# kobby-pentangeli/chaum-pedersen-zkp

Measured on AMD Instinct MI355X. Metric: verified proofs/sec (1/2/4/8 MI355X) + % int-VALU roofline vs host-CPU, higher is better.
Workload: dtype int32/int64 limbs (GF(2^255-19), radix 2^25.5)

## Files before the change

### chaum-pedersen-zkp_amd/build_native.py

```python
from __future__ import annotations

import os
import shutil
import subprocess
import sys
from concurrent.futures import ThreadPoolExecutor

PKG = os.path.dirname(os.path.abspath(__file__))
ROOT = os.path.dirname(PKG)
CSRC = os.path.join(PKG, "csrc")
LIBDIR = os.path.join(PKG, "lib")
LIBCPZ = os.path.join(LIBDIR, "libcpz.so")
HOSTTEST = os.path.join(ROOT, "tests", "native", "libcpz_hosttest.so")
DEVPROBE = os.path.join(ROOT, "tests", "native", "libcpz_devprobe.so")
ARCH = os.environ.get("CPZ_OFFLOAD_ARCH", "gfx950")


def _hipcc() -> str:
    for cand in (shutil.which("hipcc"), "/opt/rocm/bin/hipcc"):
        if cand and os.path.exists(cand):
            return cand
    raise RuntimeError("hipcc not found: the gfx950 build needs ROCm")


def _newer(out: str, srcs) -> bool:
    if not os.path.exists(out):
        return True
    t = os.path.getmtime(out)
    return any(os.path.getmtime(s) > t for s in srcs)


def _headers():
    hdr = [os.path.join(CSRC, f) for f in os.listdir(CSRC) if f.endswith(".h")]
    return hdr + [os.path.join(ROOT, "include", "cpz.h")]


def _run(cmd):
    r = subprocess.run(cmd, stdout=subprocess.PIPE, stderr=subprocess.STDOUT, text=True)
    if r.returncode != 0:
        raise RuntimeError("build step failed: %s\n%s" % (" ".join(cmd), r.stdout[-4000:]))
    return r.stdout


UNIT_FLAGS = {"wide.hip": ["-falign-loops=64"]}


def build_libcpz(force: bool = False, verbose: bool = False, out: str = LIBCPZ, defines=()) -> str:
    units = ["kernels.hip", "wide.hip", "rlc.hip", "part.hip", "runtime.hip"]
    srcs = [os.path.join(CSRC, u) for u in units] + _headers()
    if not force and not defines and not _newer(out, srcs):
        return out
    objdir = os.path.join(os.path.dirname(out), "obj" if not defines else "obj_" + "_".join(defines).replace("=", ""))
    os.makedirs(objdir, exist_ok=True)
    hipcc = _hipcc()
    common = [hipcc, "--offload-arch=" + ARCH, "-O3", "-std=c++17", "-fPIC", "-I", CSRC,
              "-I", os.path.join(ROOT, "include")] + ["-D" + d for d in defines]
    if defines and os.environ.get("CPZ_EXTRA_FLAGS"):
        common += os.environ["CPZ_EXTRA_FLAGS"].split()

    def compile_one(u):
        obj = os.path.join(objdir, u.replace(".hip", ".o"))
        if force or defines or _newer(obj, [os.path.join(CSRC, u)] + _headers()):
            uf = [] if defines and os.environ.get("CPZ_NO_UNIT_FLAGS") else UNIT_FLAGS.get(u, [])
            _run(common + uf + ["-c", os.path.join(CSRC, u), "-o", obj])
        return obj

    with ThreadPoolExecutor(max_workers=len(units)) as ex:
        objs = list(ex.map(compile_one, units))
    tmp = out + ".tmp"
    _run([hipcc, "--offload-arch=" + ARCH, "-shared", "-fPIC", "-o", tmp] + objs)
    os.replace(tmp, out)
    if verbose:
        print("built", out)
    return out


CLOCK_PROBE_LIB = os.path.join(LIBDIR, "timing", "clock_probe.so")


def build_clock_probe(force: bool = False) -> str:
    os.makedirs(os.path.dirname(CLOCK_PROBE_LIB), exist_ok=True)
    return build_libcpz(force, out=CLOCK_PROBE_LIB, defines=("CPZ_CLOCK_PROBE", "CPZ_TIMING_ONLY"))


def build_hosttest(force: bool = False) -> str:
    src = os.path.join(ROOT, "tests", "native", "hostlib.cpp")
    if not force and not _newer(HOSTTEST, [src] + _headers()):
        return HOSTTEST
    cxx = shutil.which("g++") or "g++"
    tmp = HOSTTEST + ".tmp"
    extra = ["-D" + d for d in os.environ.get("CPZ_HOST_DEFINES", "").split()]
    _run([cxx, "-O2", "-std=c++17", "-fPIC", "-shared", "-DCPZ_BOUNDS_CHECK", "-DCPZ_COUNT_OPS"] + extra +
         ["-I", CSRC, src, "-o", tmp])
    os.replace(tmp, HOSTTEST)
    return HOSTTEST


def build_devprobe(force: bool = False, out: str = DEVPROBE, include: str = CSRC) -> str:
    src = os.path.join(ROOT, "tests", "native", "devprobe.hip")
    hdrs = [os.path.join(include, f) for f in os.listdir(include) if f.endswith(".h")]
    if not force and not _newer(out, [src] + hdrs):
        return out
    tmp = out + ".tmp"
    _run([_hipcc(), "--offload-arch=" + ARCH, "-O3", "-std=c++17", "-fPIC", "-I", include,
          "-I", os.path.join(ROOT, "include"), "-shared", src, "-o", tmp])
    os.replace(tmp, out)
    return out


CPP_TEST = os.path.join(ROOT, "tests", "cpp", "batch_verifier_test")


def build_cpp_test(force: bool = False) -> str:
    src = os.path.join(ROOT, "tests", "cpp", "batch_verifier_test.cpp")
    hdrs = [os.path.join(ROOT, "include", "cpz.h"), os.path.join(ROOT, "include", "cpz_batch.hpp")]
    if not force and not _newer(CPP_TEST, [src] + hdrs):
        return CPP_TEST
    cxx = shutil.which("g++") or "g++"
    _run([cxx, "-O2", "-std=c++17", "-I", os.path.join(ROOT, "include"), src, "-o", CPP_TEST + ".tmp",
          "-L", LIBDIR, "-lcpz", "-Wl,-rpath,$ORIGIN/../../chaum-pedersen-zkp_amd/lib"])
    os.replace(CPP_TEST + ".tmp", CPP_TEST)
    return CPP_TEST


DROPIN_TEST = os.path.join(ROOT, "tests", "cpp", "dropin_test")


def build_dropin_test(force: bool = False) -> str:
    src = os.path.join(ROOT, "tests", "cpp", "dropin_test.cpp")
    hdrs = [os.path.join(ROOT, "include", "cpz.h"), os.path.join(ROOT, "include", "cpz_batch.hpp")]
    if not force and not _newer(DROPIN_TEST, [src] + hdrs):
        return DROPIN_TEST
    cxx = shutil.which("g++") or "g++"
    _run([cxx, "-O2", "-std=c++17", "-I", os.path.join(ROOT, "include"), src, "-o", DROPIN_TEST + ".tmp",
          "-L", LIBDIR, "-lcpz", "-Wl,-rpath,$ORIGIN/../../chaum-pedersen-zkp_amd/lib"])
    os.replace(DROPIN_TEST + ".tmp", DROPIN_TEST)
    return DROPIN_TEST


MERGE_TEST = os.path.join(ROOT, "tests", "cpp", "merge_groups_test")


def build_merge_groups_test(force: bool = False) -> str:
    src = os.path.join(ROOT, "tests", "cpp", "merge_groups_test.cpp")
    hdrs = [os.path.join(ROOT, "include", "cpz.h"), os.path.join(ROOT, "include", "cpz_batch.hpp")]
    if not force and not _newer(MERGE_TEST, [src] + hdrs):
        return MERGE_TEST
    cxx = shutil.which("g++") or "g++"
    _run([cxx, "-O2", "-std=c++17", "-I", os.path.join(ROOT, "include"), src, "-o", MERGE_TEST + ".tmp",
          "-L", LIBDIR, "-lcpz", "-Wl,-rpath,$ORIGIN/../../chaum-pedersen-zkp_amd/lib"])
    os.replace(MERGE_TEST + ".tmp", MERGE_TEST)
    return MERGE_TEST


def build_oracle(force: bool = False) -> None:
    mk = os.path.join(ROOT, "oracle", "Makefile")
    if os.path.exists(mk):
        _run(["make", "-s", "-C", os.path.join(ROOT, "oracle")] + (["-B"] if force else []))


def build_all(force: bool = False, verbose: bool = False) -> None:
    build_hosttest(force)
    build_oracle(force)
    build_libcpz(force, verbose)
    build_devprobe(force)
    build_cpp_test(force)
    build_dropin_test(force)
    build_merge_groups_test(force)


if __name__ == "__main__":
    build_all(force="--force" in sys.argv, verbose=True)
```

### chaum-pedersen-zkp_amd/csrc/cpz_kernels.h

```cpp
#pragma once
#include <hip/hip_runtime.h>
#include <stdint.h>

#include "scalarmul.h"

namespace cpz {

constexpr uint8_t kStatusOk = 0;
constexpr uint8_t kStatusEqFail = 1;
constexpr uint8_t kStatusBadPoint = 2;
constexpr uint8_t kStatusBadScalar = 3;
constexpr uint8_t kStatusIdentity = 4;
constexpr uint8_t kStatusZeroS = 5;

constexpr int kNielsEntries = kTableB;
constexpr int kNielsLevels = 8;
__host__ __device__ constexpr int niels_level_doublings(int level) {
  return level == 0 ? 0 : (level == 1 ? 128 : (level == 2 ? 64 : (level == 3 ? 192 : 32 * (2 * (level - 4) + 1))));
}
constexpr int kNielsLevelOfPart[8] = {0, 4, 2, 5, 1, 6, 3, 7};
constexpr bool niels_parts_consistent() {
  for (int q = 0; q < 8; q++)
    if (niels_level_doublings(kNielsLevelOfPart[q]) != 32 * q) return false;
  return true;
}
static_assert(niels_parts_consistent(), "kNielsLevelOfPart must invert niels_level_doublings");
constexpr int kCachedEntries = 2 * kTableSlots;
#ifndef CPZ_VERIFY_BLOCK
#define CPZ_VERIFY_BLOCK 256
#endif
constexpr int kVerifyBlock = CPZ_VERIFY_BLOCK;

struct StrobeSnap {
  uint8_t state[200];
  int32_t pos;
  int32_t pos_begin;
  int32_t flags;
  int32_t pad;
};

struct ChallengeArgs {
  int64_t n;
  uint32_t gh_words[16];
  const uint32_t* y1;
  const uint32_t* y2;
  const uint32_t* r1;
  const uint32_t* r2;
  const uint32_t* s;
  const uint8_t* ctx_bytes;
  const uint64_t* ctx_off;
  const uint8_t* ctx_present;
  const uint64_t* ctx_end = nullptr;
  const StrobeSnap* prefix;
  uint32_t* c_out;
  uint8_t* status_out;
  int fast_noctx = 0;
  uint32_t k1[50];
  uint32_t k2[50];
  int fast_ctx32 = 0;
  uint32_t c32[3][50];
  int eq_only = 0;
};

enum ParseCode : uint8_t {
  kParseOk = 0, kParseTooSmall, kParseBadVersion,
  kParseR1LenMissing, kParseR1LenInvalid, kParseR1Truncated, kParseR1Size, kParseR1Point,
  kParseR2LenMissing, kParseR2LenInvalid, kParseR2Truncated, kParseR2Size, kParseR2Point,
  kParseSLenMissing, kParseSLenInvalid, kParseSTruncated, kParseSSize, kParseSScalar,
  kParseTrailing, kParseIdentity, kParseZeroS
};

struct ParseArgs {
  int64_t n;
  const uint8_t* blob;
  const uint64_t* off;
  uint32_t* r1;
  uint32_t* r2;
  uint32_t* s;
  uint8_t* code;
  uint32_t* aux;
};

constexpr int kProbeChunks = 16;
struct ProbeGatherArgs {
  int64_t starts[kProbeChunks];
  int blk;
  const uint32_t* rows[5];
  uint32_t* out_rows[5];
  const uint64_t* ctx_off;
  const uint8_t* ctx_present;
  uint64_t* out_begin;
  uint64_t* out_end;
  uint8_t* out_present;
};

#ifndef CPZ_VERIFY_QUAD
#define CPZ_VERIFY_QUAD 1
#endif
#ifndef CPZ_QUAD_MAX
#define CPZ_QUAD_MAX 16384
#endif
constexpr int64_t kQuadVerifyMax = CPZ_QUAD_MAX;
constexpr int kQuadTableInts = 2 * 9 * 40;
constexpr int64_t kVarBaseMax = kQuadVerifyMax;
constexpr int kQuadPhases = 9;
constexpr int kSmallStamps = 16;
constexpr int64_t kQuadProofScratch = 2 * kQuadTableInts * 4;

struct VerifyArgs {
  int64_t n;
  const uint32_t* y1;
  const uint32_t* y2;
  const uint32_t* r1;
  const uint32_t* r2;
  const uint32_t* s;
  const uint32_t* c;
  uint8_t* status;
  const ge_niels* comb;
  char* scratch;
  const ge_niels* pre = nullptr;
  int eq_only = 0;
  const uint32_t* blocks = nullptr;
  int block_proofs = 0;
  int64_t nblocks = 0;
  int64_t quad_max = 0;
  uint64_t* clock_probe = nullptr;
  const int32_t* vtab16 = nullptr;
  const ge_niels* vtab = nullptr;
};

struct PairDesc {
  const ge_niels* tab;
  const int32_t* tab16;
  StrobeSnap prefix[2];
  uint32_t gh_words[16];
  int32_t fast_noctx;
  int32_t fast_ctx32;
  uint32_t k1[50];
  uint32_t k2[50];
  uint32_t c32[3][50];
};
static_assert(sizeof(PairDesc) % 16 == 0, "descriptor rows stay 16-byte aligned");
struct PairArgs {
  const PairDesc* desc = nullptr;
  const uint32_t* pair_idx = nullptr;
};

struct ProveArgs {
  int64_t n;
  uint64_t first_index;
  uint32_t seed_x[8];
  uint32_t seed_k[8];
  const uint32_t* x_in;
  const uint32_t* k_in;
  const ge_niels* comb;
  uint32_t* y1;
  uint32_t* y2;
  uint32_t* r1;
  uint32_t* r2;
  const uint32_t* c;
  uint32_t* s_out;
};

hipError_t launch_transcript_prefix(const uint32_t* gh_words, StrobeSnap* out, hipStream_t st);
hipError_t launch_challenge(const ChallengeArgs& a, hipStream_t st);
hipError_t launch_probe_gather(const ProbeGatherArgs& a, hipStream_t st);
bool challenge_prefix_is_fixed(const StrobeSnap& snap);
bool challenge_prefix_is_ctx32(const StrobeSnap& snap);
hipError_t launch_build_niels(const uint32_t* base_words, int nbases, ge_niels* tab, int* ok, ge_p3* bases,
                              hipStream_t st);
hipError_t launch_niels_r16(const ge_niels* tab, int32_t* out, int n, hipStream_t st);
hipError_t launch_parse_proofs(const ParseArgs& a, hipStream_t st);
hipError_t launch_build_comb(const uint32_t* gh_words, ge_p3* bases_scratch, ge_niels* comb, hipStream_t st);
hipError_t launch_verify_each(const VerifyArgs& a, int grid, hipStream_t st);
hipError_t launch_verify_small(const VerifyArgs& a, const ChallengeArgs& ca, hipStream_t st);
hipError_t launch_verify_wide(const VerifyArgs& a, const ChallengeArgs& ca, hipStream_t st);
hipError_t launch_verify_small_pairs(const VerifyArgs& a, const ChallengeArgs& ca, const PairArgs& pa, hipStream_t st);
hipError_t launch_verify_wide_pairs(const VerifyArgs& a, const ChallengeArgs& ca, const PairArgs& pa, hipStream_t st);
int verify_each_blocks_per_cu();
hipError_t launch_prove_points(const ProveArgs& a, hipStream_t st);
hipError_t launch_prove_response(const ProveArgs& a, hipStream_t st);
hipError_t launch_decode_encode(int64_t n, const uint32_t* pts, uint8_t* ok, uint32_t* out, hipStream_t st);
hipError_t launch_response_prep(int64_t n, const uint32_t* s, const uint32_t* c_in, uint32_t* c_out, uint8_t* status,
                                int eq_only, hipStream_t st);

}
```

### chaum-pedersen-zkp_amd/csrc/runtime.hip

```cpp
#include <hip/hip_runtime.h>

#include <algorithm>
#include <atomic>
#include <cstdint>
#include <cstdio>
#include <cstdlib>
#include <cstring>
#include <mutex>
#include <string>
#include <thread>
#include <vector>

#include "../../include/cpz.h"
#include "cpz_kernels.h"
#include "rlc.h"
#include "verify.h"

namespace {

thread_local std::string g_last_error;

int fail(int code, const std::string& msg) {
  g_last_error = msg;
  return code;
// ... 315 lines not shown
  static const uint8_t zero[32] = {0};
  if (std::memcmp(g, zero, 32) == 0 || std::memcmp(h, zero, 32) == 0)
    return fail(CPZ_EGENERATOR, "generator cannot be identity");
  if (std::memcmp(g, h, 32) == 0) return fail(CPZ_EGENERATOR, "generators g and h must be different");
  if (ctx->have_last) CPZ_HIP(hipEventSynchronize(ctx->last_done));
  GenSet& e = light ? *lru_victim(ctx->light, kLightCache) : *lru_victim(ctx->gen, ctx->gen_cap);
  e.valid = false;
  e.full = !light;
  if (ctx->gs == &e) ctx->gs = nullptr;
  StageTimer timer(ctx, light ? 13 : 7, ctx->stream);
  if (int rc = build_niels_prefix(ctx, e, both)) return rc;
  if (!light) {
    const size_t comb_bytes = (size_t)2 * cpz::kCombPerBase * sizeof(cpz::ge_niels);
    if (e.comb.ensure(comb_bytes) != hipSuccess) {
      (void)hipGetLastError();
      for (int k = 0; k < ctx->gen_cap; k++)
        if (&ctx->gen[k] != &e) ctx->gen[k].release();
      for (GenSet& l : ctx->light) l.release();
      CPZ_HIP(e.comb.ensure(comb_bytes));
    }
    CPZ_HIP(e.comb_q.ensure((size_t)2 * cpz::kCombWindows * sizeof(cpz::ge_p3)));
    CPZ_HIP(cpz::launch_build_comb(static_cast<const uint32_t*>(e.gh_words.p), static_cast<cpz::ge_p3*>(e.comb_q.p),
                                   static_cast<cpz::ge_niels*>(e.comb.p), ctx->stream));
    CPZ_HIP(hipStreamSynchronize(ctx->stream));
  }
  std::memcpy(e.gh, both, 64);
  e.valid = true;
  e.used = ++ctx->gen_clock;
  ctx->gs = &e;
  return CPZ_OK;
}

void set_challenge_schedules(const cpz_ctx* ctx, cpz::ChallengeArgs& ca) {
  ca.eq_only = ctx->call_eq ? 1 : 0;
  ca.fast_noctx = ctx->gs->prefix_fixed ? 1 : 0;
  std::memcpy(ca.k1, ctx->gs->chal_k1, sizeof(ca.k1));
  std::memcpy(ca.k2, ctx->gs->chal_k2, sizeof(ca.k2));
  ca.fast_ctx32 = ctx->gs->ctx32_fixed ? 1 : 0;
  std::memcpy(ca.c32, ctx->gs->chal_c32, sizeof(ca.c32));
}

int occupancy_grid(const cpz_ctx* ctx) { return ctx->cus * ctx->verify_blocks_per_cu; }

int verify_grid(cpz_ctx* ctx, size_t n) {
  const size_t want = (n + cpz::kVerifyBlock - 1) / cpz::kVerifyBlock;
  const size_t cap = (size_t)occupancy_grid(ctx);
  return (int)(want < cap ? want : cap);
}

#ifndef CPZ_VERIFY_STREAMS
#define CPZ_VERIFY_STREAMS 2
#endif
#ifndef CPZ_VERIFY_SMALL
#define CPZ_VERIFY_SMALL 1
#endif
#ifndef CPZ_SMALL_MAX
#define CPZ_SMALL_MAX 2048
#endif
constexpr int64_t kSmallMax = CPZ_SMALL_MAX;
#ifndef CPZ_WIDE_MAX
#define CPZ_WIDE_MAX 512
#endif
bool zero_copy() {
  static const bool v = [] {
    const char* e = std::getenv("CPZ_ZERO_COPY");
    return !(e && e[0] == '0');
  }();
  return v;
}
int64_t wide_max() {
  static const int64_t v = [] {
    const char* e = std::getenv("CPZ_WIDE_MAX");
    return e ? (int64_t)std::atoll(e) : (int64_t)CPZ_WIDE_MAX;
  }();
  return v;
}
#ifndef CPZ_VERIFY_CHUNK_DIV
#define CPZ_VERIFY_CHUNK_DIV 2
#endif
int verify_full_grid(const cpz_ctx* ctx) {
  return (occupancy_grid(ctx) + CPZ_VERIFY_CHUNK_DIV - 1) / CPZ_VERIFY_CHUNK_DIV;
}
size_t verify_slab_bytes(const cpz_ctx* ctx) {
  return (size_t)verify_full_grid(ctx) * cpz::kVerifyBlock * cpz::kCachedEntries * sizeof(cpz::ge_cached);
}
int64_t verify_quad_max(const cpz_ctx* ctx) {
  return std::min<int64_t>(cpz::kQuadVerifyMax, (int64_t)(verify_slab_bytes(ctx) / cpz::kQuadProofScratch));
}
int64_t var_base_max(const cpz_ctx* ctx) { return std::min<int64_t>(cpz::kVarBaseMax, verify_quad_max(ctx)); }
struct VerifyRR {
  int64_t next = 0;
};

int join_verify_streams(cpz_ctx* ctx, hipStream_t st) {
  for (int k = 0; k < CPZ_VERIFY_STREAMS - 1; k++) {
    if (!ctx->aux_stream[k]) continue;
    CPZ_HIP(hipEventRecord(ctx->aux_done[k], ctx->aux_stream[k]));
    CPZ_HIP(hipStreamWaitEvent(st, ctx->aux_done[k], 0));
  }
  return CPZ_OK;
}

int launch_verify_chunks(cpz_ctx* ctx, const cpz::VerifyArgs& va, int stage, hipStream_t st, VerifyRR* rr,
                         bool join, const cpz::ChallengeArgs* ca = nullptr, const cpz::PairArgs* pairs = nullptr) {
  static_assert(CPZ_VERIFY_STREAMS >= 1 && CPZ_VERIFY_STREAMS <= 4, "1..4 verify streams");
  const int full = verify_full_grid(ctx);
  const int grid = std::min(full, verify_grid(ctx, (size_t)va.n));
  const size_t slab = verify_slab_bytes(ctx);
  const int64_t per = (int64_t)grid * cpz::kVerifyBlock;
  const int64_t chunks = (va.n + per - 1) / per;
  const int nst = rr ? CPZ_VERIFY_STREAMS : (int)std::min<int64_t>(CPZ_VERIFY_STREAMS, chunks);
  CPZ_HIP(ctx->scratch.ensure((size_t)CPZ_VERIFY_STREAMS * slab));
  if (nst > 1) {
    if (!ctx->aux_start) CPZ_HIP(hipEventCreateWithFlags(&ctx->aux_start, hipEventDisableTiming));
    CPZ_HIP(hipEventRecord(ctx->aux_start, st));
    for (int k = 0; k < nst - 1; k++) {
      if (!ctx->aux_stream[k]) CPZ_HIP(stream_own_queue(&ctx->aux_stream[k], ctx->cus, ctx->device, &ctx->own_queues));
      if (!ctx->aux_done[k]) CPZ_HIP(hipEventCreateWithFlags(&ctx->aux_done[k], hipEventDisableTiming));
      CPZ_HIP(hipStreamWaitEvent(ctx->aux_stream[k], ctx->aux_start, 0));
    }
  }
  for (int64_t c = 0; c < chunks; c++) {
    const int64_t a = c * per;
    cpz::VerifyArgs v = va;
    v.n = (va.n - a) < per ? (va.n - a) : per;
    v.y1 = va.y1 + 8 * a;
    v.y2 = va.y2 + 8 * a;
    v.r1 = va.r1 + 8 * a;
    v.r2 = va.r2 + 8 * a;
    v.s = va.s + 8 * a;
    v.c = va.c + 8 * a;
    if (va.pre) v.pre = va.pre + 4 * a;
    v.status = va.status + a;
    v.quad_max = verify_quad_max(ctx);
#if defined(CPZ_CLOCK_PROBE)
    CPZ_HIP(ctx->clk[3].ensure(cpz::kSmallStamps * sizeof(uint64_t)));
    ctx->clk_waves[3] = 1;
    v.clock_probe = static_cast<uint64_t*>(ctx->clk[3].p);
#endif
    const int k = (int)((rr ? rr->next++ : c) % nst);
    v.scratch = static_cast<char*>(ctx->scratch.p) + (size_t)k * slab;
    hipStream_t sc = k == 0 ? st : ctx->aux_stream[k - 1];
    if (CPZ_VERIFY_SMALL && v.n <= kSmallMax && !v.pre && !v.blocks && (!ca || !ca->ctx_end)) {
      cpz::ChallengeArgs cc{};
      if (ca) {
        cc = *ca;
        cc.n = v.n;
        if (ca->ctx_off) cc.ctx_off = ca->ctx_off + a;
        if (ca->ctx_present) cc.ctx_present = ca->ctx_present + a;
        v.c = nullptr;
      }
      StageTimer t(ctx, stage, sc);
      if (pairs) {
        cpz::PairArgs pp = *pairs;
        pp.pair_idx += a;
        if (v.n <= wide_max())
          CPZ_HIP(cpz::launch_verify_wide_pairs(v, cc, pp, sc));
        else
          CPZ_HIP(cpz::launch_verify_small_pairs(v, cc, pp, sc));
      } else if (v.n <= wide_max()) {
        CPZ_HIP(cpz::launch_verify_wide(v, cc, sc));
      } else {
        CPZ_HIP(cpz::launch_verify_small(v, cc, sc));
      }
      continue;
    }
    if (pairs) return fail(CPZ_EINVAL, "internal: mixed-pair call outside the latency kernels' range");
// ... 1937 lines not shown
```

### chaum-pedersen-zkp_amd/csrc/scalar25519.h

```cpp
#pragma once
#include <math.h>

#include "fe25519.h"

namespace cpz {

struct sc {
  uint32_t w[8];
};

CPZ_HD uint32_t SC_L(int i) {
  const uint32_t l[8] = {0x5cf5d3edu, 0x5812631au, 0xa2f79cd6u, 0x14def9deu,
                         0x00000000u, 0x00000000u, 0x00000000u, 0x10000000u};
  return l[i];
}

CPZ_HD uint32_t SC_MU(int i) {
  const uint32_t mu[9] = {0x0a2c131bu, 0xed9ce5a3u, 0x086329a7u, 0x2106215du, 0xffffffebu,
                          0xffffffffu, 0xffffffffu, 0xffffffffu, 0x0000000fu};
  return mu[i];
}

CPZ_HD bool sc_geq_l9(const uint32_t a[9]) {
  if (a[8] != 0) return true;
// ... 418 lines not shown
      const int32_t u2 = u0 - (int32_t)q * u1, v2 = v0 - (int32_t)q * v1;
      const int32_t au2 = u2 < 0 ? -u2 : u2, av2 = v2 < 0 ? -v2 : v2;
      const int32_t au1 = u1 < 0 ? -u1 : u1, av1 = v1 < 0 ? -v1 : v1;
      const uint32_t e2 = (uint32_t)(au2 + av2) + 1, e1 = (uint32_t)(au1 + av1) + 1;
      const bool go = (B != 0u) & (qe < (1u << 15)) & (au2 < (1 << 15)) & (av2 < (1 << 15)) & (R >= e2 + tsh) &
                      (B - R >= e1 + e2);
      if (!go) break;
      A = B;
      B = R;
      u0 = u1;
      v0 = v1;
      u1 = u2;
      v1 = v2;
      steps++;
    }
    if (steps == 0) {
      half_split_step(r0, r1, t0, t1);
    } else {
#if defined(__HIP_DEVICE_COMPILE__)
      if constexpr (kLanes) {
        const int k = (int)(threadIdx.x & 3);
        const int32_t cu = (k & 1) ? u1 : u0, cv = (k & 1) ? v1 : v0;
        const bool pos = cu > 0 || cv < 0;
        const uint32_t au = (uint32_t)(cu < 0 ? -cu : cu), av = (uint32_t)(cv < 0 ? -cv : cv);
        uint32_t X[8], Y[8], out[8];
#pragma unroll
        for (int j = 0; j < 8; j++) {
          const uint32_t x = (k & 2) ? t0[j] : r0[j], y = (k & 2) ? t1[j] : r1[j];
          X[j] = pos ? x : y;
          Y[j] = pos ? y : x;
        }
        words8_mulsub2(out, pos ? au : av, X, pos ? av : au, Y);
#pragma unroll
        for (int j = 0; j < 8; j++) {
          r0[j] = __builtin_amdgcn_readlane(out[j], 0);
          r1[j] = __builtin_amdgcn_readlane(out[j], 1);
          t0[j] = __builtin_amdgcn_readlane(out[j], 2);
          t1[j] = __builtin_amdgcn_readlane(out[j], 3);
        }
        continue;
      }
#endif
      uint32_t nr0[8], nr1[8], nt0[8], nt1[8];
      words8_row(nr0, u0, v0, r0, r1);
      words8_row(nr1, u1, v1, r0, r1);
      words8_row(nt0, u0, v0, t0, t1);
      words8_row(nt1, u1, v1, t0, t1);
#pragma unroll
      for (int j = 0; j < 8; j++) {
        r0[j] = nr0[j];
        r1[j] = nr1[j];
        t0[j] = nt0[j];
        t1[j] = nt1[j];
      }
    }
  }
  vneg = (t1[7] >> 31) != 0;
  uint32_t borrow = 0;
#pragma unroll
  for (int j = 0; j < 4; j++) {
    u[j] = r1[j];
    const uint64_t d = (uint64_t)0 - t1[j] - borrow;
    borrow = (uint32_t)(d >> 63);
    vabs[j] = vneg ? (uint32_t)d : t1[j];
  }
}

CPZ_HD void sc_recode_radix16_half(uint32_t out[4], const uint32_t s[4]) {
  int32_t carry = 0;
#pragma unroll
  for (int j = 0; j < 4; j++) {
    uint32_t packed = 0;
#pragma unroll
    for (int m = 0; m < 8; m++) {
      const int32_t n = (int32_t)((s[j] >> (4 * m)) & 15u) + carry;
      carry = (n + 8) >> 4;
      const int32_t d = n - (carry << 4);
      packed |= ((uint32_t)d & 15u) << (4 * m);
    }
    out[j] = packed;
  }
}

}
```

### chaum-pedersen-zkp_amd/csrc/scalarmul.h

```cpp
#pragma once
#include "timing_only.h"
#include "ristretto.h"

namespace cpz {

constexpr int kTableV = 8;
constexpr int kTableSlots = kTableV + 1;
constexpr int kTableB = 128;

constexpr int kCombWindows = 16;
constexpr int kCombEntries = 1 << 15;
constexpr int kCombStride = kCombEntries + 1;
constexpr int64_t kCombPerBase = (int64_t)kCombWindows * kCombStride;

struct CombTable {
  const ge_niels* p;
  CPZ_HDM ge_niels lookup(int k, int digit) const {
    const int mag = digit < 0 ? -digit : digit;
    const ge_niels* e = p + (int64_t)k * kCombStride + mag;
    ge_niels r;
#if defined(__HIP_DEVICE_COMPILE__)
    const uint4* s = reinterpret_cast<const uint4*>(e);
    uint4* d = reinterpret_cast<uint4*>(&r);
#pragma unroll
    for (int v = 0; v < (int)(sizeof(ge_niels) / 16); v++) d[v] = s[v];
#else
    r = *e;
#endif
    return ge_niels_cneg(r, digit < 0);
  }
};

constexpr int kCachedVecs = (int)(sizeof(ge_cached) / 16);

struct SlabTable {
  char* base;
  uint32_t col;
  static constexpr uint32_t kEntryBytes = kCachedVecs * 16;
  CPZ_HDM const char* entry(int e) const { return base + (col + (uint32_t)e * kEntryBytes); }
  CPZ_HDM SlabTable shifted(int e0) const { return SlabTable{base, col + (uint32_t)e0 * kEntryBytes}; }
  CPZ_HDM ge_cached load(int e) const {
    ge_cached r;
    uint32_t* d = reinterpret_cast<uint32_t*>(&r);
    const char* p = entry(e);
#pragma unroll
    for (int v = 0; v < kCachedVecs; v++) {
#if defined(__HIP_DEVICE_COMPILE__)
      const uint4 x = *reinterpret_cast<const uint4*>(p + 16 * v);
      d[4 * v] = x.x; d[4 * v + 1] = x.y; d[4 * v + 2] = x.z; d[4 * v + 3] = x.w;
#else
      const uint32_t* s = reinterpret_cast<const uint32_t*>(p + 16 * v);
      for (int k = 0; k < 4; k++) d[4 * v + k] = s[k];
#endif
    }
    return r;
  }
  CPZ_HDM void store(int e, const ge_cached& c) const {
    const uint32_t* s = reinterpret_cast<const uint32_t*>(&c);
    char* p = const_cast<char*>(entry(e));
#pragma unroll
    for (int v = 0; v < kCachedVecs; v++) {
#if defined(__HIP_DEVICE_COMPILE__)
      *reinterpret_cast<uint4*>(p + 16 * v) = make_uint4(s[4 * v], s[4 * v + 1], s[4 * v + 2], s[4 * v + 3]);
#else
      uint32_t* d = reinterpret_cast<uint32_t*>(p + 16 * v);
      for (int k = 0; k < 4; k++) d[k] = s[4 * v + k];
#endif
    }
  }
};

struct DigitRef {
  const uint32_t* p;
  int stride;
  CPZ_HDM uint32_t operator[](int k) const { return p[k * stride]; }
};
CPZ_HD DigitRef host_digits(const uint32_t* a) { return DigitRef{a, 1}; }

CPZ_HD SlabTable host_table(ge_cached* p) { return SlabTable{reinterpret_cast<char*>(p), 0u}; }

CPZ_HD ge_niels niels_lookup(const ge_niels* tab, int digit) {
  const int mag = digit < 0 ? -digit : digit;
  const ge_niels e = tab[(mag == 0 ? 1 : mag) - 1];
  const ge_niels r = mag == 0 ? ge_niels_identity() : e;
  return ge_niels_cneg(r, digit < 0);
}

CPZ_HD ge_cached cached_lookup(const SlabTable& tab, int digit) {
  const int mag = digit < 0 ? -digit : digit;
  return ge_cached_cneg(tab.load(mag), digit < 0);
}
CPZ_HD ge_p1p1 dbl4(const ge_p1p1& cur) {
  ge_p1p1 t = cur;
#pragma unroll 1
  for (int d = 0; d < 4; d++) t = p2_dbl(p1p1_to_p2(t));
  return t;
}

CPZ_HD ge_p1p1 p1p1_identity() {
  ge_p1p1 cur;
  cur.X = fe_zero(); cur.Y = fe_one(); cur.Z = fe_one(); cur.T = fe_one();
  return cur;
}

CPZ_HD void build_cached_table(const SlabTable& tab, const ge_p3& P) {
  ge_niels n1;
  n1.ypx = fe_add(P.Y, P.X);
  n1.ymx = fe_sub(P.Y, P.X);
  n1.xy2d = fe_mul(P.T, FE_D2());
  tab.store(0, ge_cached_identity());
  {
    ge_cached c1;
    c1.YpX = n1.ypx;
    c1.YmX = n1.ymx;
    c1.Z = P.Z;
    c1.T2d = n1.xy2d;
    tab.store(1, c1);
  }
  ge_p3 acc = p1p1_to_p3(p3_dbl(P));
  tab.store(2, p3_to_cached(acc));
#pragma unroll 1
  for (int k = 3; k <= kTableV; k++) {
    acc = p1p1_to_p3(ge_add_niels(acc, n1));
    tab.store(k, p3_to_cached(acc));
  }
}

CPZ_HD ge_p3 straus_vartime(const SlabTable& tab_v, const ge_niels* tab_b, const uint32_t cdig_in[8],
                            const uint32_t sdig_in[8]) {
  uint32_t cdig[8], sdig[8];
#pragma unroll
  for (int j = 0; j < 8; j++) { cdig[j] = cdig_in[j]; sdig[j] = sdig_in[j]; }
  ge_p1p1 cur = p1p1_identity();
#pragma unroll 1
  for (int j = 7; j >= 0; j--) {
    const uint32_t wc = cdig[7], wg = sdig[7];
#pragma unroll
    for (int t = 7; t > 0; t--) { cdig[t] = cdig[t - 1]; sdig[t] = sdig[t - 1]; }
#pragma unroll 1
    for (int m = 7; m >= 0; m--) {
      const int dc = ((int32_t)(wc << (28 - 4 * m))) >> 28;
      const ge_cached ev = cached_lookup(tab_v, dc);
      if (j != 7 || m != 7) cur = dbl4(cur);
      cur = ge_add_cached(p1p1_to_p3(cur), ev);
      if ((m & 1) == 0) {
        const int dg = ((int32_t)(wg << (24 - 8 * (m >> 1)))) >> 24;
        cur = ge_add_niels(p1p1_to_p3(cur), niels_lookup(tab_b, dg));
      }
    }
  }
  return p1p1_to_p3(cur);
}

template <class Comb, class Dig>
CPZ_HD ge_p1p1 comb_add(ge_p1p1 cur, const Comb& comb, const Dig& sd) {
#pragma unroll 1
  for (int j = 0; j < 8; j++) {
    const uint32_t w = sd[j];
#pragma unroll
    for (int m = 0; m < 2; m++) {
      const int d = (int32_t)(w << (16 - 16 * m)) >> 16;
      cur = ge_add_niels(p1p1_to_p3(cur), comb.lookup(2 * j + m, d));
    }
  }
  return cur;
}

template <class Comb, class Dig>
CPZ_HD ge_p1p1 straus_half_comb(const SlabTable& tab_y, const SlabTable& tab_r, const Comb& comb, const Dig& ud,
                              const Dig& vd, const Dig& sdig) {
  ge_p1p1 cur = p1p1_identity();
#pragma unroll 1
  for (int j = 3; j >= 0; j--) {
    const uint32_t wu = ud[j], wv = vd[j];
#pragma unroll 1
    for (int m = 7; m >= 0; m--) {
      const int du = ((int32_t)(wu << (28 - 4 * m))) >> 28;
      const int dv = ((int32_t)(wv << (28 - 4 * m))) >> 28;
      const ge_cached ey = cached_lookup(tab_y, du), er = cached_lookup(tab_r, dv);
      if (j != 3 || m != 7) cur = dbl4(cur);
#if defined(CPZ_EXP_NIELS_TABLES)
      cur = ge_add_niels(p1p1_to_p3(cur), ge_niels{ey.YpX, ey.YmX, ey.T2d, {0, 0}});
      cur = ge_add_niels(p1p1_to_p3(cur), ge_niels{er.YpX, er.YmX, er.T2d, {0, 0}});
#else
      cur = ge_add_cached(p1p1_to_p3(cur), ey);
      cur = ge_add_cached(p1p1_to_p3(cur), er);
#endif
    }
  }
  return comb_add(cur, comb, sdig);
}

template <class Comb>
CPZ_HD ge_p3 comb_mul(const Comb& comb, const uint32_t sdig[8]) {
  return p1p1_to_p3(comb_add(p1p1_identity(), comb, host_digits(sdig)));
}

CPZ_HD ge_p3 fixed_base_mul(const ge_niels* tab_b, const uint32_t sdig_in[8]) {
  uint32_t sdig[8];
#pragma unroll
  for (int j = 0; j < 8; j++) sdig[j] = sdig_in[j];
  ge_p1p1 cur = p1p1_identity();
#pragma unroll 1
  for (int j = 7; j >= 0; j--) {
    const uint32_t wg = sdig[7];
#pragma unroll
    for (int t = 7; t > 0; t--) sdig[t] = sdig[t - 1];
#pragma unroll 1
    for (int m = 3; m >= 0; m--) {
      if (j != 7 || m != 3) {
        cur = dbl4(cur);
        cur = dbl4(cur);
      }
      const int dg = ((int32_t)(wg << (24 - 8 * m))) >> 24;
      cur = ge_add_niels(p1p1_to_p3(cur), niels_lookup(tab_b, dg));
    }
  }
  return p1p1_to_p3(cur);
}

CPZ_HD ge_p3 small_mul(const ge_p3& B, int k) {
  ge_p3 acc = ge_identity();
#pragma unroll 1
  for (int bit = 7; bit >= 0; bit--) {
    acc = p1p1_to_p3(p3_dbl(acc));
    if ((k >> bit) & 1) acc = ge_add(acc, B);
  }
  return acc;
}

}
```

### chaum-pedersen-zkp_amd/csrc/verify.h

```cpp
#pragma once
#include "timing_only.h"
#include "ristretto.h"
#include "scalar25519.h"
#include "scalarmul.h"
#include "transcript.h"

#define CPZ_EQ_LOOP _Pragma("unroll 1")

namespace cpz {

constexpr uint8_t kStOk = 0, kStEqFail = 1, kStBadPoint = 2, kStBadScalar = 3, kStIdentity = 4, kStZeroS = 5;
constexpr uint8_t kStBadChallenge = 0x80;

CPZ_HD bool words8_zero(const uint32_t w[8]) {
  uint32_t acc = 0;
#pragma unroll
  for (int k = 0; k < 8; k++) acc |= w[k];
  return acc == 0;
}

CPZ_HD uint8_t response_status(const uint32_t s[8], bool eq_only = false) {
  if (!sc_is_canonical(s)) return kStBadScalar;
  if (sc_is_zero(s) && !eq_only) return kStZeroS;
  return kStOk;
// ... 105 lines not shown

CPZ_HD bool challenge_masks(uint32_t k1[50], uint32_t k2[50]) {
  MaskState ms;
  for (int g = 0; g < 3; g++)
    for (int i = 0; i < 200; i++) ms.m[g][i] = 0;
  Strobe<MaskState> s(ms, kTailPrefixPos, kTailPrefixBegin, (uint8_t)kTailPrefixFlags);
  const uint32_t z[8] = {0, 0, 0, 0, 0, 0, 0, 0};
  (void)transcript_challenge(s, z, z, z, z);
  if (ms.seg != 2) return false;
  for (int w = 0; w < 50; w++) {
    uint32_t a = 0, b = 0;
    for (int k = 3; k >= 0; k--) {
      a = (a << 8) | ms.m[0][4 * w + k];
      b = (b << 8) | ms.m[1][4 * w + k];
    }
    k1[w] = a;
    k2[w] = b;
  }
  return true;
}

template <class Acc>
CPZ_HD Strobe<Acc> transcript_new(Acc& st) {
  Strobe<Acc> s = strobe_init_merlin(st);
  s.merlin_header("dom-sep", 7, 25);
  s.absorb((const uint8_t*)"Chaum-Pedersen ZKP v1.0.0", 25);
  s.merlin_header("protocol", 8, 27);
  s.absorb((const uint8_t*)"chaum-pedersen-ristretto255", 27);
  return s;
}

template <class Acc>
CPZ_HD void transcript_context(Strobe<Acc>& s, const uint8_t* ctx, uint32_t len) {
  s.merlin_header("context", 7, len);
  for (uint32_t b = 0; b < len; b++) s.absorb_byte(ctx[b]);
}

template <class Acc>
CPZ_HD void transcript_parameters(Strobe<Acc>& s, const uint32_t g[8], const uint32_t h[8]) {
  s.merlin_append_words("generator-g", 11, g);
  s.merlin_append_words("generator-h", 11, h);
}

CPZ_HD bool challenge_masks_ctx32(uint32_t m[3][50], const uint32_t g[8], const uint32_t h[8]) {
  MaskState ms;
  for (int k = 0; k < 3; k++)
    for (int i = 0; i < 200; i++) ms.m[k][i] = 0;
  Strobe<MaskState> s(ms, kC32PrefixPos, kC32PrefixBegin, (uint8_t)kC32PrefixFlags);
  const uint8_t zc[32] = {0};
  const uint32_t z[8] = {0, 0, 0, 0, 0, 0, 0, 0};
  transcript_context(s, zc, 32);
  transcript_parameters(s, g, h);
  (void)transcript_challenge(s, z, z, z, z);
  if (ms.seg != 3) return false;
  for (int k = 0; k < 3; k++) mask_words(m[k], ms.m[k]);
  return true;
}

CPZ_HD ge_p3 affine_from_neg_niels(const ge_niels& q) {
  ge_p3 P;
  P.X = fe_mul(fe_sub(q.ymx, q.ypx), FE_INV2());
  P.Y = fe_mul(fe_add(q.ypx, q.ymx), FE_INV2());
  P.Z = fe_one();
  P.T = fe_mul(P.X, P.Y);
  return P;
}

CPZ_HD ge_niels niels_load(const ge_niels* p) {
  ge_niels r;
#if defined(__HIP_DEVICE_COMPILE__)
  const uint4* s = reinterpret_cast<const uint4*>(p);
  uint4* d = reinterpret_cast<uint4*>(&r);
#pragma unroll
  for (int v = 0; v < (int)(sizeof(ge_niels) / 16); v++) d[v] = s[v];
#else
  r = *p;
#endif
  return r;
}

template <bool kPre, class Comb, class Dig>
CPZ_HD bool check_equation(const Dig& y, const Dig& r, const ge_niels* pre_y, const ge_niels* pre_r,
                           const Dig& udig, const Dig& vdig, bool vneg, const Dig& sdig, const Comb& comb,
                           const SlabTable& tab_y, const SlabTable& tab_r, bool& decoded, bool& r_identity) {
  decoded = true;
CPZ_EQ_LOOP
  for (int k = 0; k < 2; k++) {
    ge_p3 P;
    if constexpr (kPre) {
      P = affine_from_neg_niels(niels_load(k ? pre_r : pre_y));
    } else {
      uint32_t w[8];
#pragma unroll
      for (int q = 0; q < 8; q++) w[q] = k ? r[q] : y[q];
      decoded = ristretto_decode(P, w) && decoded;
    }
    build_cached_table(k ? tab_r : tab_y, (k && vneg) ? P : ge_neg(P));
  }
  if constexpr (kPre) {
    r_identity = false;
  } else {
    uint32_t acc = 0;
#pragma unroll
    for (int q = 0; q < 8; q++) acc |= r[q];
    r_identity = acc == 0;
  }
#if defined(CPZ_EXP_EXTRA_INV)
  ge_p1p1 q = straus_half_comb(tab_y, tab_r, comb, udig, vdig, sdig);
  q.X = fe_mul(q.X, fe_invert(q.Z));
  return ristretto_is_identity(q);
#else
  return ristretto_is_identity(straus_half_comb(tab_y, tab_r, comb, udig, vdig, sdig));
#endif
}

template <bool kPre = false, class Comb>
CPZ_HD uint8_t verify_proof(const DigitRef& y1, const DigitRef& y2, const DigitRef& r1, const DigitRef& r2,
                            const uint32_t s[8], const uint32_t c[8], uint8_t st_s, const Comb& comb_g,
                            const Comb& comb_h, const SlabTable& tab_v, uint32_t* dig, int dstride,
                            const ge_niels* pre = nullptr, bool eq_only = false) {
  bool vneg;
#if defined(CPZ_EXP_NOSPLIT)
  vneg = c[7] & 1;
  for (int k = 0; k < 8; k++) {
    dig[k * dstride] = c[k];
    dig[(8 + k) * dstride] = s[k];
  }
  if (0)
#endif
  {
    uint32_t u[4], va[4], w[8];
    sc_half_split(c, u, va, vneg);
    sc_recode_radix16_half(w, u);
    sc_recode_radix16_half(w + 4, va);
    for (int k = 0; k < 8; k++) dig[k * dstride] = w[k];
    sc vs, ss;
#pragma unroll
    for (int k = 0; k < 8; k++) {
      vs.w[k] = k < 4 ? va[k] : 0u;
      ss.w[k] = s[k];
    }
    sc sp = sc_mul(vs, ss);
    if (vneg) sp = sc_neg(sp);
    sc_recode_radix65536(w, sp.w);
    for (int k = 0; k < 8; k++) dig[(8 + k) * dstride] = w[k];
  }
  const DigitRef udig{dig, dstride}, vdig{dig + 4 * dstride, dstride}, sdig{dig + 8 * dstride, dstride};
  bool dec = true, id = false, eq = true;
CPZ_EQ_LOOP
  for (int e = 0; e < 2; e++) {
    bool d, r_id;
    eq = check_equation<kPre>(e ? y2 : y1, e ? r2 : r1, kPre ? pre + 1 + 2 * e : nullptr, kPre ? pre + 2 * e : nullptr,
                              udig, vdig, vneg, sdig, e ? comb_h : comb_g, tab_v, tab_v.shifted(kTableSlots), d,
                              r_id) && eq;
    dec = dec && d;
    id = id || r_id;
  }
  if (!dec) return kStBadPoint;
  if (st_s == kStBadScalar) return kStBadScalar;
  if (id && !eq_only) return kStIdentity;
  if (st_s == kStZeroS) return kStZeroS;
  if (st_s == kStBadChallenge) return kStBadScalar;
  return eq ? kStOk : kStEqFail;
}

}
```

Before: 52.19 million.

## Replace two radix-16 Straus tables with a joint radix-4 Shamir table

The half-width Straus loop now uses one 13-entry joint table of combinations aY+bR (digits in -2..2) with radix-4 signed recoding, in place of two separate 8-entry radix-16 tables. Each window does two doublings and a single cached addition instead of four doublings and two additions. The aim is fewer point additions per scalar bit and a smaller table build. The cost is more loop iterations, a more involved table construction with extra adds and doublings, and a slab size that is now the maximum of the quad scratch and the joint table size.

```diff
diff --git a/chaum-pedersen-zkp_amd/build_native.py b/chaum-pedersen-zkp_amd/build_native.py
--- a/chaum-pedersen-zkp_amd/build_native.py
+++ b/chaum-pedersen-zkp_amd/build_native.py
@@ -84,14 +84,14 @@
 
 
 def build_hosttest(force: bool = False) -> str:
-    src = os.path.join(ROOT, "tests", "native", "hostlib.cpp")
-    if not force and not _newer(HOSTTEST, [src] + _headers()):
+    srcs = [os.path.join(ROOT, "tests", "native", f) for f in ("hostlib.cpp", "hostlib_joint.cpp")]
+    if not force and not _newer(HOSTTEST, srcs + _headers()):
         return HOSTTEST
     cxx = shutil.which("g++") or "g++"
     tmp = HOSTTEST + ".tmp"
     extra = ["-D" + d for d in os.environ.get("CPZ_HOST_DEFINES", "").split()]
     _run([cxx, "-O2", "-std=c++17", "-fPIC", "-shared", "-DCPZ_BOUNDS_CHECK", "-DCPZ_COUNT_OPS"] + extra +
-         ["-I", CSRC, src, "-o", tmp])
+         ["-I", CSRC] + srcs + ["-o", tmp])
     os.replace(tmp, HOSTTEST)
     return HOSTTEST
 
diff --git a/chaum-pedersen-zkp_amd/csrc/cpz_kernels.h b/chaum-pedersen-zkp_amd/csrc/cpz_kernels.h
--- a/chaum-pedersen-zkp_amd/csrc/cpz_kernels.h
+++ b/chaum-pedersen-zkp_amd/csrc/cpz_kernels.h
@@ -25,7 +25,7 @@
   return true;
 }
 static_assert(niels_parts_consistent(), "kNielsLevelOfPart must invert niels_level_doublings");
-constexpr int kCachedEntries = 2 * kTableSlots;
+constexpr int kCachedEntries = kJointSlots;
 #ifndef CPZ_VERIFY_BLOCK
 #define CPZ_VERIFY_BLOCK 256
 #endif
@@ -106,6 +106,9 @@
 constexpr int kQuadPhases = 9;
 constexpr int kSmallStamps = 16;
 constexpr int64_t kQuadProofScratch = 2 * kQuadTableInts * 4;
+constexpr int64_t kSlabThreadBytes =
+    kQuadProofScratch / 2 > (int64_t)(kCachedEntries * sizeof(ge_cached)) ? kQuadProofScratch / 2
+                                                                          : (int64_t)(kCachedEntries * sizeof(ge_cached));
 
 struct VerifyArgs {
   int64_t n;
diff --git a/chaum-pedersen-zkp_amd/csrc/runtime.hip b/chaum-pedersen-zkp_amd/csrc/runtime.hip
--- a/chaum-pedersen-zkp_amd/csrc/runtime.hip
+++ b/chaum-pedersen-zkp_amd/csrc/runtime.hip
@@ -421,7 +421,7 @@
   return (occupancy_grid(ctx) + CPZ_VERIFY_CHUNK_DIV - 1) / CPZ_VERIFY_CHUNK_DIV;
 }
 size_t verify_slab_bytes(const cpz_ctx* ctx) {
-  return (size_t)verify_full_grid(ctx) * cpz::kVerifyBlock * cpz::kCachedEntries * sizeof(cpz::ge_cached);
+  return (size_t)verify_full_grid(ctx) * cpz::kVerifyBlock * (size_t)cpz::kSlabThreadBytes;
 }
 int64_t verify_quad_max(const cpz_ctx* ctx) {
   return std::min<int64_t>(cpz::kQuadVerifyMax, (int64_t)(verify_slab_bytes(ctx) / cpz::kQuadProofScratch));
diff --git a/chaum-pedersen-zkp_amd/csrc/scalar25519.h b/chaum-pedersen-zkp_amd/csrc/scalar25519.h
--- a/chaum-pedersen-zkp_amd/csrc/scalar25519.h
+++ b/chaum-pedersen-zkp_amd/csrc/scalar25519.h
@@ -524,4 +524,29 @@
   }
 }
 
-}
+CPZ_HD void sc_recode_radix4_half(uint32_t out[4], const uint32_t s[4]) {
+  CPZ_ASSERT(s[3] < 0x60000000u);
+  int32_t carry = 0;
+#pragma unroll
+  for (int j = 0; j < 4; j++) {
+    uint32_t packed = 0;
+#pragma unroll
+    for (int m = 0; m < 16; m++) {
+      const int32_t n = (int32_t)((s[j] >> (2 * m)) & 3u) + carry;
+      if (j == 3 && m == 15) {
+        CPZ_ASSERT(n <= 2);
+        carry = 0;
+        packed |= (uint32_t)n << 30;
+      } else {
+        carry = (n + 2) >> 2;
+        packed |= ((uint32_t)(n - (carry << 2)) & 3u) << (2 * m);
+      }
+    }
+    out[j] = packed;
+  }
+}
+
+CPZ_HD int radix4_digit(uint32_t w, int m) { return ((int32_t)(w << (30 - 2 * m))) >> 30; }
+CPZ_HD int radix4_top_digit(uint32_t w3) { return (int)(w3 >> 30); }
+
+}
diff --git a/chaum-pedersen-zkp_amd/csrc/scalarmul.h b/chaum-pedersen-zkp_amd/csrc/scalarmul.h
--- a/chaum-pedersen-zkp_amd/csrc/scalarmul.h
+++ b/chaum-pedersen-zkp_amd/csrc/scalarmul.h
@@ -1,6 +1,7 @@
 #pragma once
 #include "timing_only.h"
 #include "ristretto.h"
+#include "scalar25519.h"
 
 namespace cpz {
 
@@ -166,25 +167,69 @@
   return cur;
 }
 
+constexpr int kJointSlots = 13;
+CPZ_HD constexpr int joint_slot(int a, int b) { return 5 * a + b; }
+CPZ_HD int joint_window(uint32_t wu, uint32_t wv, int m) { return joint_slot(radix4_digit(wu, m), radix4_digit(wv, m)); }
+CPZ_HD int joint_top_window(uint32_t wu3, uint32_t wv3) {
+  return joint_slot(radix4_top_digit(wu3), radix4_top_digit(wv3));
+}
+
+CPZ_HD void build_joint_table(const SlabTable& tab, const ge_p3& Y, const ge_p3& R) {
+  ge_niels nY, nR;
+  nY.ypx = fe_add(Y.Y, Y.X);
+  nY.ymx = fe_sub(Y.Y, Y.X);
+  nY.xy2d = fe_mul(Y.T, FE_D2());
+  nR.ypx = fe_add(R.Y, R.X);
+  nR.ymx = fe_sub(R.Y, R.X);
+  nR.xy2d = fe_mul(R.T, FE_D2());
+  tab.store(0, ge_cached_identity());
+  tab.store(joint_slot(1, 0), ge_cached{nY.ypx, nY.ymx, Y.Z, nY.xy2d});
+  tab.store(joint_slot(0, 1), ge_cached{nR.ypx, nR.ymx, R.Z, nR.xy2d});
+#pragma unroll 1
+  for (int neg = 0; neg < 2; neg++) {
+    const int s = neg ? -1 : 1;
+    const ge_niels nRs = ge_niels_cneg(nR, neg != 0);
+    ge_p3 A = Y;
+#pragma unroll 1
+    for (int j = 0; j < 3; j++) {
+      const ge_p3 Q = p1p1_to_p3(ge_add_niels(A, j == 2 ? nY : nRs));
+      tab.store(j == 0 ? joint_slot(1, s) : (j == 1 ? joint_slot(1, 2 * s) : joint_slot(2, s)), p3_to_cached(Q));
+      if (j == 0) A = Q;
+    }
+#pragma unroll 1
+    for (int d = 0; d < 2; d++) {
+      const ge_p3& P = d == 0 ? A : (neg ? R : Y);
+      const int slot = d == 0 ? joint_slot(2, 2 * s) : (neg ? joint_slot(0, 2) : joint_slot(2, 0));
+      tab.store(slot, p3_to_cached(p1p1_to_p3(p2_dbl(ge_p2{P.X, P.Y, P.Z}))));
+    }
+  }
+}
+
+CPZ_HD ge_p1p1 cached_to_p1p1(const ge_cached& e) {
+  ge_p1p1 r;
+  r.X = fe_sub(e.YpX, e.YmX);
+  r.Y = fe_add(e.YpX, e.YmX);
+  r.Z = fe_add(e.Z, e.Z);
+  r.T = r.Z;
+  return r;
+}
+
 template <class Comb, class Dig>
-CPZ_HD ge_p1p1 straus_half_comb(const SlabTable& tab_y, const SlabTable& tab_r, const Comb& comb, const Dig& ud,
-                              const Dig& vd, const Dig& sdig) {
-  ge_p1p1 cur = p1p1_identity();
+CPZ_HD ge_p1p1 straus_half_joint(const SlabTable& tab, const Comb& comb, const Dig& ud, const Dig& vd,
+                                 const Dig& sdig) {
+  ge_p1p1 cur = cached_to_p1p1(tab.load(joint_top_window(ud[3], vd[3])));
 #pragma unroll 1
   for (int j = 3; j >= 0; j--) {
     const uint32_t wu = ud[j], wv = vd[j];
 #pragma unroll 1
-    for (int m = 7; m >= 0; m--) {
-      const int du = ((int32_t)(wu << (28 - 4 * m))) >> 28;
-      const int dv = ((int32_t)(wv << (28 - 4 * m))) >> 28;
-      const ge_cached ey = cached_lookup(tab_y, du), er = cached_lookup(tab_r, dv);
-      if (j != 3 || m != 7) cur = dbl4(cur);
+    for (int m = j == 3 ? 14 : 15; m >= 0; m--) {
+      const ge_cached e = cached_lookup(tab, joint_window(wu, wv, m));
+      cur = p2_dbl(p1p1_to_p2(cur));
+      cur = p2_dbl(p1p1_to_p2(cur));
 #if defined(CPZ_EXP_NIELS_TABLES)
-      cur = ge_add_niels(p1p1_to_p3(cur), ge_niels{ey.YpX, ey.YmX, ey.T2d, {0, 0}});
-      cur = ge_add_niels(p1p1_to_p3(cur), ge_niels{er.YpX, er.YmX, er.T2d, {0, 0}});
-#else
-      cur = ge_add_cached(p1p1_to_p3(cur), ey);
-      cur = ge_add_cached(p1p1_to_p3(cur), er);
+      cur = ge_add_niels(p1p1_to_p3(cur), ge_niels{e.YpX, e.YmX, e.T2d, {0, 0}});
+#else
+      cur = ge_add_cached(p1p1_to_p3(cur), e);
 #endif
     }
   }
diff --git a/chaum-pedersen-zkp_amd/csrc/verify.h b/chaum-pedersen-zkp_amd/csrc/verify.h
--- a/chaum-pedersen-zkp_amd/csrc/verify.h
+++ b/chaum-pedersen-zkp_amd/csrc/verify.h
@@ -211,8 +211,9 @@
 template <bool kPre, class Comb, class Dig>
 CPZ_HD bool check_equation(const Dig& y, const Dig& r, const ge_niels* pre_y, const ge_niels* pre_r,
                            const Dig& udig, const Dig& vdig, bool vneg, const Dig& sdig, const Comb& comb,
-                           const SlabTable& tab_y, const SlabTable& tab_r, bool& decoded, bool& r_identity) {
+                           const SlabTable& tab, bool& decoded, bool& r_identity) {
   decoded = true;
+  ge_p3 Yp, Rp;
 CPZ_EQ_LOOP
   for (int k = 0; k < 2; k++) {
     ge_p3 P;
@@ -224,8 +225,10 @@
       for (int q = 0; q < 8; q++) w[q] = k ? r[q] : y[q];
       decoded = ristretto_decode(P, w) && decoded;
     }
-    build_cached_table(k ? tab_r : tab_y, (k && vneg) ? P : ge_neg(P));
-  }
+    P = (k && vneg) ? P : ge_neg(P);
+    if (k) Rp = P; else Yp = P;
+  }
+  build_joint_table(tab, Yp, Rp);
   if constexpr (kPre) {
     r_identity = false;
   } else {
@@ -235,11 +238,11 @@
     r_identity = acc == 0;
   }
 #if defined(CPZ_EXP_EXTRA_INV)
-  ge_p1p1 q = straus_half_comb(tab_y, tab_r, comb, udig, vdig, sdig);
+  ge_p1p1 q = straus_half_joint(tab, comb, udig, vdig, sdig);
   q.X = fe_mul(q.X, fe_invert(q.Z));
   return ristretto_is_identity(q);
 #else
-  return ristretto_is_identity(straus_half_comb(tab_y, tab_r, comb, udig, vdig, sdig));
+  return ristretto_is_identity(straus_half_joint(tab, comb, udig, vdig, sdig));
 #endif
 }
 
@@ -252,7 +255,7 @@
 #if defined(CPZ_EXP_NOSPLIT)
   vneg = c[7] & 1;
   for (int k = 0; k < 8; k++) {
-    dig[k * dstride] = c[k];
+    dig[k * dstride] = k % 4 == 3 ? c[k] & 0x3fffffffu : c[k];
     dig[(8 + k) * dstride] = s[k];
   }
   if (0)
@@ -260,8 +263,8 @@
   {
     uint32_t u[4], va[4], w[8];
     sc_half_split(c, u, va, vneg);
-    sc_recode_radix16_half(w, u);
-    sc_recode_radix16_half(w + 4, va);
+    sc_recode_radix4_half(w, u);
+    sc_recode_radix4_half(w + 4, va);
     for (int k = 0; k < 8; k++) dig[k * dstride] = w[k];
     sc vs, ss;
 #pragma unroll
@@ -280,8 +283,7 @@
   for (int e = 0; e < 2; e++) {
     bool d, r_id;
     eq = check_equation<kPre>(e ? y2 : y1, e ? r2 : r1, kPre ? pre + 1 + 2 * e : nullptr, kPre ? pre + 2 * e : nullptr,
-                              udig, vdig, vneg, sdig, e ? comb_h : comb_g, tab_v, tab_v.shifted(kTableSlots), d,
-                              r_id) && eq;
+                              udig, vdig, vneg, sdig, e ? comb_h : comb_g, tab_v, d, r_id) && eq;
     dec = dec && d;
     id = id || r_id;
   }
```

New measurement: 53.36 million (median of 6 runs). +2.2%, better.
